# samholt/NeuralLaplaceControl

Hardware: AMD Instinct MI355X
Metric: MPPI planning steps/sec (16384 samples, H=40) (higher is better)
Workload: dtype f64

## Files before the change

neurallaplacecontrol_amd/csrc/abi_ctx.hip:

```cpp
#include "nlc_host.h"

using namespace nlc;
using namespace nlc::host;

namespace nlc {
namespace host {

thread_local std::string g_create_error;

bool gru_use_coop(const nlc_ctx* c, int64_t n_windows) {
  if (c->opt.gru_coop >= 0) return c->opt.gru_coop != 0;
  if (c->g == 128) return true;
  return n_windows <= (c->g == 32 ? 8192 : 50000);
}

void prof_flush(nlc_ctx* c) {
  for (auto& p : c->prof) {
    for (auto& ev : p.pending) {
      hipEventSynchronize(ev.second);
      float ms = 0.f;
      hipEventElapsedTime(&ms, ev.first, ev.second);
      p.total_ms += ms;
      c->event_pool.push_back(ev.first);
      c->event_pool.push_back(ev.second);
// ... 157 lines not shown
    if (value < 0 || value > 3) return fail(c, NLC_ERR_BAD_ARG, "fused_inline must be 0, 1 (= 3), or the bit mask 1 weights | 2 sampling");
    c->opt.fused_inline = (int)value == 1 ? 3 : (int)value;
  } else if (n == "fused_spin_limit") {
    if (value < 1 || value > 4.0e9) return fail(c, NLC_ERR_BAD_ARG, "fused_spin_limit must be in 1 .. 4e9");
    c->opt.fused_spin_limit = (int64_t)value;
  } else if (n == "linear_fused") {
    c->opt.linear_fused = value != 0.0;
  } else if (n == "test_lin_coeff_scale") {
    c->opt.test_lin_coeff_scale = value;
    c->has_mppi = false;
  } else if (n == "fused_keep_sync") {
    c->opt.fused_keep_sync = value != 0.0;
  } else if (n == "fused_test_drop_tile") {
    if (value < -1) return fail(c, NLC_ERR_BAD_ARG, "fused_test_drop_tile must be >= -1");
    c->opt.fused_test_drop_tile = (int)value;
  } else if (n == "fused_roll_cap") {
    if (value < 0) return fail(c, NLC_ERR_BAD_ARG, "fused_roll_cap must be >= 0 (0 = auto)");
    c->opt.fused.roll_cap = (int)value;
  } else if (n == "fused_chain_first_tiles") {
    if (value < -1 || value > 64) return fail(c, NLC_ERR_BAD_ARG, "fused_chain_first_tiles must be in -1..64 (-1 = auto)");
    c->opt.fused.chain_first_tiles = (int)value;
  } else if (n == "fused_partner_tiles") {
    if (value < -2 || value > 64) return fail(c, NLC_ERR_BAD_ARG, "fused_partner_tiles must be in -2..64 (-2 = auto, -1 = never)");
    c->opt.fused.partner_tiles = (int)value;
  } else if (n == "repfunc_split") {
    if (value != 0 && value != 1) return fail(c, NLC_ERR_BAD_ARG, "repfunc_split must be 0 or 1");
    c->opt.repfunc_split = (int)value;
  } else if (n == "gru_coop") {
    if (value != 0 && value != 1 && value != -1) return fail(c, NLC_ERR_BAD_ARG, "gru_coop must be -1 (auto), 0 or 1");
    c->opt.gru_coop = (int)value;
  } else if (n == "gru_prefix") {
    if (value != 0 && value != 1 && value != -1) return fail(c, NLC_ERR_BAD_ARG, "gru_prefix must be -1 (auto), 0 or 1");
    c->opt.gru_prefix = (int)value;
  } else if (n == "gru_gemm") {
    if (value != 0 && value != 1) return fail(c, NLC_ERR_BAD_ARG, "gru_gemm must be 0 (FP64 MFMA) or 1 (int8-sliced)");
    c->opt.gru_gemm = (int)value;
    if (c->has_model) c->gru.use_i8 = (c->gru.i8_stream != nullptr && value == 1) ? 1 : 0;
  } else if (n == "dbg_gap_us") {
    if (value < 0 || value > 1.0e5) return fail(c, NLC_ERR_BAD_ARG, "dbg_gap_us must be in 0 .. 1e5");
    c->opt.dbg_gap_us = value;
  } else if (n == "dbg_l2_mb") {
    if (value < 0 || value > 4096) return fail(c, NLC_ERR_BAD_ARG, "dbg_l2_mb must be in 0 .. 4096");
    c->opt.dbg_l2_mb = value;
  } else if (n == "fused_max_samples") {
    if (value < 0) return fail(c, NLC_ERR_BAD_ARG, "fused_max_samples must be >= 0");
    c->opt.fused_max_samples = (int64_t)value;
  } else {
    return fail(c, NLC_ERR_BAD_ARG, "unknown option: " + n);
  }
  return NLC_OK;
}

extern "C" int nlc_get_stat(nlc_ctx* c, const char* name, double* out) {
  if (!c) return NLC_ERR_BAD_ARG;
  if (!name || !out) return fail(c, NLC_ERR_BAD_ARG, "NULL stat name / out");
  const std::string n(name);
  if (n == "rollout_body") *out = (double)c->last_body;
  else if (n == "fused_timeouts") *out = (double)c->fused.timeouts;
  else if (n == "fused_fallbacks") *out = (double)c->fused.fallbacks;
  else if (n == "fused_lost") *out = c->fused.lost ? 1.0 : 0.0;
  else if (n == "last_giveup_command") *out = (double)c->fused.last_giveup_command;
  else if (n == "commands") *out = (double)c->commands;
  else if (n == "comm_world") *out = c->comm ? (double)c->comm_world : 0.0;
  else if (n == "comm_rank") *out = c->comm ? (double)c->comm_rank : -1.0;
  else if (n == "fused_blocks_per_cu") *out = (double)c->fused.blocks_per_cu;
  else if (n == "fused_spin_limit") *out = (double)c->opt.fused_spin_limit;
  else if (n == "model_nt3") *out = c->has_model ? (double)c->net.nt3 : 0.0;
  else if (n == "gru_gemm") *out = (c->has_model && c->gru.use_i8) ? 1.0 : 0.0;
  else if (n == "gru_prefix") *out = c->prefix.last_used ? 1.0 : 0.0;
  else if (n.rfind("gru_prefix_windows_l", 0) == 0 && n.size() == 21 && n[20] >= '0' && n[20] <= '4') {
    *out = 0.0;
    if (c->prefix.last_used && c->prefix.lists) {
      unsigned cnt[nlc::prefix::kLists] = {0};
      NLC_HIP(c, hipStreamSynchronize(c->stream));
      NLC_HIP(c, hipMemcpy(cnt, c->prefix.lists, sizeof(cnt), hipMemcpyDeviceToHost));
      *out = (double)cnt[n[20] - '0'];
    }
  } else if (n == "gru_prefix_table_tiles") {
    *out = 0.0;
    if (c->prefix.last_used && c->prefix.lists) {
      unsigned cnt[nlc::prefix::kLists] = {0};
      NLC_HIP(c, hipStreamSynchronize(c->stream));
      NLC_HIP(c, hipMemcpy(cnt, c->prefix.lists, sizeof(cnt), hipMemcpyDeviceToHost));
      for (int l = 1; l < nlc::prefix::n_lists(c->prefix.last_B); ++l) *out += (double)((cnt[l] + 15u) / 16u);
    }
  } else if (n == "latents_offset") *out = (c->has_mppi && c->pd.dynamics == NLC_DYN_NL) ? (double)ws_layout(c).pa : -1.0;
  else if (n == "gru_i8_launches") *out = (double)nlc::gru_i8_launch_count();
  else return fail(c, NLC_ERR_BAD_ARG, "unknown stat: " + n);
  return NLC_OK;
}

extern "C" int nlc_synchronize(nlc_ctx* c) {
  if (!c) return NLC_ERR_BAD_ARG;
  NLC_HIP(c, hipStreamSynchronize(c->stream));
  return NLC_OK;
}

extern "C" int nlc_device_info(nlc_ctx* c, char* name, int name_len, int* cus, int* mhz, double* gib) {
  if (!c) return NLC_ERR_BAD_ARG;
  if (name && name_len > 0) {
    std::snprintf(name, name_len, "%s (%s)", c->prop.name, c->prop.gcnArchName);
  }
  if (cus) *cus = c->prop.multiProcessorCount;
  if (mhz) *mhz = c->prop.clockRate / 1000;
  if (gib) *gib = (double)c->prop.totalGlobalMem / (1024.0 * 1024.0 * 1024.0);
  return NLC_OK;
}

extern "C" int nlc_profile_enable(nlc_ctx* c, int on) {
  if (!c) return NLC_ERR_BAD_ARG;
  if (!on) prof_flush(c);
  c->profiling = on != 0;
  return NLC_OK;
}
extern "C" int nlc_profile_reset(nlc_ctx* c) {
  if (!c) return NLC_ERR_BAD_ARG;
// ... 19 lines not shown
```

neurallaplacecontrol_amd/csrc/abi_planner.hip:

```cpp
#include "nlc_host.h"

using namespace nlc;
using namespace nlc::host;

extern "C" int nlc_mppi_configure(nlc_ctx* c, const nlc_mppi_desc* d) {
  if (!c) return NLC_ERR_BAD_ARG;
  NLC_GUARD_BEGIN
  if (!d) return fail(c, NLC_ERR_BAD_ARG, "NULL desc");
  if (d->K < 1 || d->T < 1 || d->K_global < d->K || d->k_offset < 0 || d->k_offset + d->K > d->K_global)
    return fail(c, NLC_ERR_BAD_SHAPE, "bad K / K_global / k_offset / T");
  if (d->nu < 1 || d->nu > NLC_MAX_NU) return fail(c, NLC_ERR_UNSUPPORTED, "nu must be 1 or 2");
  if (d->d < 1 || (d->d > NLC_MAX_D && d->dynamics != NLC_DYN_EXTERNAL)) return fail(c, NLC_ERR_BAD_SHAPE, "bad nx");
  if (d->B < 1) return fail(c, NLC_ERR_BAD_SHAPE, "action_buffer needs at least one row");
  if (!(d->lambda_ > 0.0) || d->u_scale == 0.0) return fail(c, NLC_ERR_BAD_ARG, "lambda_ must be > 0, u_scale != 0");
  if (d->u_per_command < 1 || d->u_per_command > d->T) return fail(c, NLC_ERR_BAD_ARG, "bad u_per_command");
  if (d->E < 0 || d->E > 65535) return fail(c, NLC_ERR_BAD_ARG, "episodes E must be in [0, 65535]");
  const int E = d->E < 1 ? 1 : d->E;
  if ((double)E * (double)d->K * d->T * d->nu > 2.0e9)
    return fail(c, NLC_ERR_BAD_SHAPE, "E*K*T*nu exceeds the planner's index range");
  const bool env_free = d->cost_external &&
                        (d->dynamics == NLC_DYN_NL || d->dynamics == NLC_DYN_DTRNN || d->dynamics == NLC_DYN_NODE) &&
                        d->env == -1;
  if (!env_free && (d->env < 0 || d->env > NLC_ENV_CARTPOLE_NOTRIG)) return fail(c, NLC_ERR_UNSUPPORTED, "unknown env id");
  static const int env_d[4] = {5, 3, 6, 4}, env_nu[4] = {1, 1, 2, 1};
// ... 162 lines not shown
  wa.nblk = c->nblk;
  return wa;
}

int finish_rollout_costs(nlc_ctx* c, const nlc_mppi_buffers* buf, bool in_body) {
  const nlc_mppi_desc& d = c->pd;
  if (d.cost_external) return NLC_OK;
  if (cost_variant_of(d) && !in_body) {
    if (!buf->states) return fail(c, NLC_ERR_BAD_ARG, "this rollout body evaluates a cost_variant on buf->states");
    VariantCostArgs v{d.K * d.E, d.T, d.nu, d.d, d.env, cost_variant_of(d), d.u_scale, buf->states, buf->perturbed, buf->cost_total};
    ProfScope ps(c, "variant_cost_kernel");
    NLC_HIP(c, launch_variant_cost(v, c->stream));
  }
  return run_weights(c, buf);
}

int run_weights(nlc_ctx* c, const nlc_mppi_buffers* buf) {
  WeightArgs wa = make_weight_args(c, buf);
  if (c->last_body == 3 && buf->workspace && c->pd.dynamics == NLC_DYN_NL)
    wa.gave_up = reinterpret_cast<const unsigned*>((const double*)buf->workspace + ws_layout(c).sync) + kFusedTimeout;
  ProfScope ps(c, "weight_kernels");
  NLC_HIP(c, launch_weights(wa, c->stream));
  return NLC_OK;
}

int launch_shift_perturb(nlc_ctx* c, RolloutCall& call) {
  PerturbArgs& p = call.p;
  p.fused_shift = (int64_t)p.K * p.T > 0;
  if (!p.fused_shift) {
    ProfScope ps(c, "shift_U_kernel");
    NLC_HIP(c, launch_shift_U(p, c->stream));
  }
  ProfScope ps(c, "perturb_kernel");
  NLC_HIP(c, launch_perturb(p, c->stream));
  return NLC_OK;
}

SampleCostArgs sample_cost_args(const nlc_ctx* c, const RolloutCall& call) {
  const nlc_mppi_desc& d = c->pd;
  SampleCostArgs a{};
  a.K = call.KE;
  a.Kep = d.K;
  a.T = d.T;
  a.nu = d.nu;
  a.env = (d.cost_external || cost_variant_of(d)) ? -1 : d.env;
  a.state_per_sample = call.state_per_sample;
  a.state0 = call.state_dev;
  a.perturbed = call.buf->perturbed;
  a.noise = call.buf->noise;
  a.U = c->U[c->ucur];
  for (int i = 0; i < NLC_MAX_NU * NLC_MAX_NU; ++i) a.sigma_inv[i] = d.noise_sigma_inv[i];
  a.lambda_ = d.lambda_;
  a.u_scale = d.u_scale;
  a.noise_abs_cost = d.noise_abs_cost;
  a.states = call.buf->states;
  a.cost_total = call.buf->cost_total;
  return a;
}

PerturbArgs perturb_args(const nlc_ctx* c, const nlc_mppi_buffers* buf, int rng, uint64_t seed, uint64_t counter) {
  const nlc_mppi_desc& d = c->pd;
  PerturbArgs p{};
  p.K = d.K * d.E;
  p.Kep = d.K;
  p.E = d.E;
  p.K_global = d.K_global;
  p.k_offset = d.k_offset;
// ... 390 lines not shown
```

neurallaplacecontrol_amd/csrc/abi_planner_nl.hip:

```cpp
#include "nlc_host.h"

using namespace nlc;
using namespace nlc::host;

namespace {

__global__ void dbg_spin_kernel(unsigned long long ticks_100mhz) {
  const unsigned long long t0 = __builtin_amdgcn_s_memrealtime();
  while (__builtin_amdgcn_s_memrealtime() - t0 < ticks_100mhz) __builtin_amdgcn_s_sleep(8);
}
__global__ void dbg_touch_kernel(const double* __restrict__ p, size_t n, double* __restrict__ sink) {
  double acc = 0.0;
  for (size_t i = (size_t)blockIdx.x * blockDim.x + threadIdx.x; i < n; i += (size_t)gridDim.x * blockDim.x) acc += p[i];
  if (acc == 12345.678) *sink = acc;
}
int dbg_between(nlc_ctx* c) {
  if (c->opt.dbg_gap_us > 0.0) hipLaunchKernelGGL(dbg_spin_kernel, dim3(1), dim3(64), 0, c->stream, (unsigned long long)(c->opt.dbg_gap_us * 100.0));
  if (c->opt.dbg_l2_mb > 0.0) {
    const size_t bytes = (size_t)(c->opt.dbg_l2_mb * 1048576.0);
    const size_t n = bytes / 8 + 1;
    if (c->dbg_scratch_n < n) {
      if (int rc = hold_doubles(c, c->dbg_scratch, n, nullptr, &c->dbg_scratch_n)) return rc;
      NLC_HIP(c, hipMemsetAsync(c->dbg_scratch, 0, n * sizeof(double), c->stream));
    }
// ... 296 lines not shown
  fc.n_enc = s.n_enc;
  fc.roll_cap = s.roll_cap;
  fc.adaptive_q8 = s.adaptive_q8;
  fc.pool_wgs = s.pool_wgs;
  fc.chain_first_tiles = s.chain_first_tiles;
  fc.partner_tiles = s.partner_tiles;
  fc.spin_limit = (unsigned)c->opt.fused_spin_limit;
  fc.test_drop_tile = c->opt.fused_test_drop_tile;
  fc.inline_weights = (c->opt.fused_inline & 1) && d.E == 1 && !d.cost_external;
  fc.inline_perturb = (c->opt.fused_inline & 2) && d.E == 1 && inline_inputs && rng == 1 && d.B <= kFusedMaxInlineB;
  unsigned* sync_words = reinterpret_cast<unsigned*>(ws + w.sync);
  const size_t n_sync = fused_sync_words(d.T, KE);
  if (fc.inline_perturb) {
    if (c->fused.sync_clean_ws != buf->workspace) NLC_HIP(c, hipMemsetAsync(sync_words, 0, n_sync * sizeof(unsigned), c->stream));
  } else {
    p.zero_words = sync_words;
    p.n_zero_words = (int64_t)n_sync;
    if (int rc = launch_shift_perturb(c, call)) return rc;
  }
  c->fused.sync_clean_ws = nullptr;
  c->fused.sync_dirty = true;
  c->fused.last.fused = true;
  c->last_body = 3;
  f.p = p;
  if (fc.inline_weights) f.w = make_weight_args(c, buf);
  {
    ProfScope ps(c, "nl_plan_fused_kernel");
    NLC_HIP(c, launch_nl_plan_fused(f, c->g, s.grid, s.built, c->stream));
  }
  *weights_done = fc.inline_weights != 0;
  return NLC_OK;
}

int gru_prefix_begin(nlc_ctx* c, RolloutCall& call, const GruArgs& g, int64_t N, int chunks, bool* use, GruPrefixArgs* px) {
  *use = false;
  if (c->opt.gru_prefix == 0) return NLC_OK;
  GruPrefixState& ps = c->prefix;
  const char* why = ps.why_not;
  if (!why && ps.last_B != g.B) why = "gru_prefix: the table was built for another action-buffer length";
  if (!why && chunks != 1) why = "gru_prefix: not with the encoder in horizon chunks (horizon_chunks)";
  if (!why && gru_use_coop(c, N)) why = "gru_prefix: this launch takes the cooperative encoder (gru_coop)";
  if (!why && g.use_i8) why = "gru_prefix: the FP64 encoder only (gru_gemm is 1)";
  if (!why) why = prefix::out_of_scope(g.nact, g.nin, 1, g.B, N, true);
  if (why) return c->opt.gru_prefix == 1 ? fail(c, NLC_ERR_UNSUPPORTED, why) : NLC_OK;
  const int64_t stride = (N + 63) / 64 * 64;
  const size_t need = 64 + (size_t)prefix::kLists * (size_t)stride / 2;
  if (need > ps.lists_n) {
    NLC_HIP(c, hipStreamSynchronize(c->stream));
    if (int rc = hold_doubles(c, ps.lists, need, nullptr, &ps.lists_n)) return rc;
  }
  double* base = c->arena.base + ps.arena_off;
  px->table = base;
  px->out_tab = base + (size_t)prefix::kEntries * 2 * c->g;
  px->products = base + gru_prefix_products_off(c->g);
  px->counts = reinterpret_cast<unsigned*>(ps.lists);
  px->lists = reinterpret_cast<unsigned*>(ps.lists + 64);
  px->list_stride = stride;
  px->img_max = ps.img_max;
  px->img_min = ps.img_min;
  call.p.zero_words = px->counts;
  call.p.n_zero_words = 16;
  *use = true;
  return NLC_OK;
}

int rollout_nl_two_launch(nlc_ctx* c, RolloutCall& call, GruArgs& g, RolloutArgs& r, int variant) {
  const nlc_mppi_desc& d = c->pd;
  const int64_t KE = call.KE;
  bool use_prefix = false;
  GruPrefixArgs px{};
  {
    const int chunks = plan::horizon_chunks((variant != 2 && KE > 8192 && d.E == 1) ? c->opt.horizon_chunks : 1, d.T).C;
    if (int rc = gru_prefix_begin(c, call, g, KE * d.T, chunks, &use_prefix, &px)) return rc;
  }
  if (int rc2 = nlc::host::launch_shift_perturb(c, call)) return rc2;
  const plan::Chunks ck = plan::horizon_chunks((variant != 2 && KE > 8192 && d.E == 1) ? c->opt.horizon_chunks : 1, d.T);
  const int C = ck.C, Tc = ck.Tc;
  if (C == 1) {
    g.t0 = 0;
    g.Tc = d.T;
    g.N = KE * d.T;
    if (use_prefix) {
      {
        ProfScope ps(c, "gru_prefix_index_kernel");
        NLC_HIP(c, launch_gru_prefix_index(g, px, c->stream));
      }
      ProfScope ps(c, "gru_encode_kernel");
      NLC_HIP(c, launch_gru_encode_prefix(g, px, c->g, c->stream));
      c->prefix.last_used = true;
    } else {
      ProfScope ps(c, "gru_encode_kernel");
      NLC_HIP(c, launch_gru_encode(g, c->g, c->stream, gru_use_coop(c, g.N)));
    }
    if (c->opt.dbg_gap_us > 0.0 || c->opt.dbg_l2_mb > 0.0)
      if (int rc3 = dbg_between(c)) return rc3;
    r.t_begin = 0;
    r.t_end = d.T;
    ProfScope ps(c, "nl_rollout_kernel");
    NLC_HIP(c, launch_nl_rollout(r, c->stream, variant));
  } else {
    if (int rc = gru_encode_chunks(c, g, KE, C, Tc, false, 0u)) return rc;
    for (int ch = 0; ch < C; ++ch) {
      r.t_begin = ch * Tc;
      r.t_end = (r.t_begin + Tc <= d.T) ? r.t_begin + Tc : d.T;
      if (r.t_begin >= r.t_end) break;
      NLC_HIP(c, hipStreamWaitEvent(c->stream, c->side.ev_gru[ch], 0));
      ProfScope ps(c, "nl_rollout_kernel");
      NLC_HIP(c, launch_nl_rollout(r, c->stream, 1));
    }
  }
  return NLC_OK;
}

}

int nlc::host::gru_prefix_configure(nlc_ctx* c) {
  const nlc_mppi_desc& d = c->pd;
  GruPrefixState& ps = c->prefix;
  ps.last_B = d.B;
  ps.last_used = false;
  const double img[2] = {prefix::bound_image(d.u_max[0], d.u_scale), prefix::bound_image(d.u_min[0], d.u_scale)};
  bool finite = true;
// ... 109 lines not shown
```

neurallaplacecontrol_amd/csrc/kernels_gru.hip:

```cpp
#include "nlc_device.h"
#include "nlc_gru_prefix.h"
#include "nlc_gru_tile.h"
#include "nlc_kernels.h"

namespace nlc {

template <int G>
__global__ __launch_bounds__(256, G <= 64 ? 2 : 1) void gru_encode_kernel(const GruArgs a) {
  constexpr int KS = G / 4;
  const int lane = threadIdx.x & 63, wave = threadIdx.x >> 6;
  const int q = lane >> 4, c = lane & 15;
  const int64_t w = ((int64_t)blockIdx.x * 4 + wave) * 16 + c;
  const bool valid = w < a.N;
  const int64_t wc = valid ? w : a.N - 1;
  int64_t kk = 0;
  int tt = 0;
  if (a.mode == 1) {
    kk = wc / a.Tc;
    tt = a.t0 + (int)(wc - kk * a.Tc);
  }
  __shared__ double Hs[4][2][KS * 64];
  const double o = gru_encode_tile<G>(a, lane, wc, kk, tt, Hs[wave][0], Hs[wave][1]);
  if (valid && q < 2) {
    const int64_t wo = (a.mode == 1) ? kk * a.T + tt : w;
// ... 105 lines not shown
  __syncthreads();
  if (threadIdx.x <= prefix::kMaxLen) {
    const unsigned n = cnt[threadIdx.x];
    base[threadIdx.x] = n ? atomicAdd(px.counts + threadIdx.x, n) : 0u;
    cnt[threadIdx.x] = 0u;
  }
  __syncthreads();
#pragma unroll
  for (int it = 0; it < kIndexPerThread; ++it) {
    const int64_t w = w0 + it * 256;
    const int len = (int)(cls[it] & 7u);
    for (int l = 0; l < nl; ++l) {
      const unsigned long long m = __ballot(len == l);
      if (m == 0ull) continue;
      const int leader = __ffsll((long long)m) - 1;
      unsigned b = 0u;
      if (lane == leader) b = atomicAdd(&cnt[l], (unsigned)__popcll(m));
      b = (unsigned)__shfl((int)b, leader);
      if (len == l) {
        const unsigned pos = base[l] + b + (unsigned)__popcll(m & ((1ull << lane) - 1ull));
        if ((int64_t)pos < px.list_stride) px.lists[(int64_t)l * px.list_stride + pos] = (unsigned)w | ((cls[it] >> 3) << prefix::kPatternShift);
      }
    }
  }
}

template <int G>
__global__ __launch_bounds__(256, G <= 64 ? 2 : 1) void gru_encode_prefix_kernel(const GruArgs a, const GruPrefixArgs px) {
  constexpr int KS = G / 4;
  const int lane = threadIdx.x & 63;
  const int wave = __builtin_amdgcn_readfirstlane(threadIdx.x >> 6);
  const int q = lane >> 4, c = lane & 15;
  const int nl = prefix::n_lists(a.B);
  int64_t tile = (int64_t)blockIdx.x * 4 + wave;
  int len = 0;
  unsigned n = 0u;
  for (; len < nl; ++len) {
    n = px.counts[len];
    if ((int64_t)n > px.list_stride) n = (unsigned)px.list_stride;
    const int64_t nt = ((int64_t)n + 15) / 16;
    if (tile < nt) break;
    tile -= nt;
  }
  if (len == nl) return;
  const int64_t idx = tile * 16 + c;
  const bool valid = idx < (int64_t)n;
  const unsigned e = px.lists[(int64_t)len * px.list_stride + (valid ? idx : (int64_t)n - 1)];
  int64_t w = (int64_t)(e & ((1u << prefix::kPatternShift) - 1u));
  if (w >= a.N) w = a.N - 1;
  const int64_t kk = w / a.Tc;
  const int tt = a.t0 + (int)(w - kk * a.Tc);
  __shared__ double Hs[4][2][KS * 64];
  double* prod = nullptr;
  if (len > 0) {
    const int pattern = (int)(e >> prefix::kPatternShift) & ((1 << len) - 1);
    const int entry = prefix::entry_index(len, pattern);
    const double* ent = px.table + (size_t)entry * 2 * G;
    prod = px.products + prefix::products_entry_offset(entry, G);
#pragma unroll
    for (int ks = 0; ks < KS; ++ks) {
      Hs[wave][0][ks * 64 + lane] = ent[4 * ks + q];
      Hs[wave][1][ks * 64 + lane] = ent[G + 4 * ks + q];
    }
  }
  const double o = gru_encode_tile<G, kTileFromTable>(a, lane, w, kk, tt, Hs[wave][0], Hs[wave][1], len, -1, prod);
  if (valid && q < 2) a.out[(kk * a.T + tt) * 2 + q] = o;
// ... 121 lines not shown
```

neurallaplacecontrol_amd/csrc/kernels_mppi.hip:

```cpp
#include "nlc_device.h"
#include "nlc_env_dev.h"
#include "nlc_envcost.h"
#include "nlc_kernels.h"
#include "nlc_mppi_dev.h"

namespace nlc {

__global__ void shift_U_kernel(const PerturbArgs a) {
  const int n = a.T * a.nu;
  const double* Uo = a.U_old + (int64_t)blockIdx.x * n;
  double* Un = a.U_new + (int64_t)blockIdx.x * n;
  for (int i = threadIdx.x; i < n; i += blockDim.x) {
    const int t = i / a.nu, j = i - t * a.nu;
    Un[i] = (t + 1 < a.T) ? Uo[i + a.nu] : a.u_init[j];
  }
  if (blockIdx.x == 0) {
    for (int i = threadIdx.x; i < a.n_state_in; i += blockDim.x) a.state_dst[i] = a.state_in[i];
    for (int i = threadIdx.x; i < a.n_abuf_in; i += blockDim.x) a.abuf_dst[i] = a.abuf_in[i];
  }
}
hipError_t launch_shift_U(const PerturbArgs& a, hipStream_t s) {
  hipLaunchKernelGGL(shift_U_kernel, dim3((unsigned)a.E), dim3(128), 0, s, a);
  return hipGetLastError();
}

__global__ __launch_bounds__(256) void perturb_kernel(const PerturbArgs a) {
  const int64_t total = a.K * a.T;
  for (int64_t i = (int64_t)blockIdx.x * blockDim.x + threadIdx.x; i < a.n_zero_words; i += (int64_t)gridDim.x * blockDim.x)
    a.zero_words[i] = 0u;
  if (a.fused_shift && blockIdx.x == 0) {
    for (int i = threadIdx.x; i < a.n_state_in; i += blockDim.x) a.state_dst[i] = a.state_in[i];
    for (int i = threadIdx.x; i < a.n_abuf_in; i += blockDim.x) a.abuf_dst[i] = a.abuf_in[i];
  }
  for (int64_t idx = (int64_t)blockIdx.x * blockDim.x + threadIdx.x; idx < total;
       idx += (int64_t)gridDim.x * blockDim.x) {
    const int64_t k = idx / a.T;
    const int t = (int)(idx - k * a.T);
    const int64_t e = k / a.Kep;
    const int64_t ke = a.k_offset + (k - e * a.Kep);
    const int64_t kg = e * a.K_global + ke;
    double eps[NLC_MAX_NU];
    if (a.rng) {
      mppi_draw(kg, t, a.seed, a.counter, a.nu, a.mu, a.chol, eps);
    } else {
      for (int i = 0; i < a.nu; ++i) eps[i] = a.noise[idx * a.nu + i];
    }
    const bool null_action = a.sample_null_action && (ke == a.K_global - 1);
    for (int i = 0; i < a.nu; ++i) {
      double U;
      if (a.fused_shift) {
        U = (t + 1 < a.T) ? a.U_old[(e * a.T + t + 1) * a.nu + i] : a.u_init[i];
        if (k == e * a.Kep) a.U_new[(e * a.T + t) * a.nu + i] = U;
      } else {
        U = a.U_new[(e * a.T + t) * a.nu + i];
      }
      const double V = mppi_bound(U, eps[i], null_action, a.u_scale, a.has_bounds, a.u_min[i], a.u_max[i]);
      a.perturbed[idx * a.nu + i] = V;
      a.noise[idx * a.nu + i] = V - U;
      if (a.actions != nullptr) a.actions[idx * a.nu + i] = (a.u_scale * V) / a.u_scale;
    }
  }
}
hipError_t launch_perturb(const PerturbArgs& a, hipStream_t s) {
  const int64_t total = a.K * a.T;
  if (total <= 0) return hipSuccess;
  const int64_t want = (total + 255) / 256;
  const unsigned grid = (unsigned)(want < 4096 ? want : 4096);
  hipLaunchKernelGGL(perturb_kernel, dim3(grid), dim3(256), 0, s, a);
  return hipGetLastError();
}

__global__ __launch_bounds__(256) void weight_tile_kernel(const WeightArgs a) {
  const int lane = threadIdx.x & 63;
  const int64_t b = (int64_t)blockIdx.x * 4 + (threadIdx.x >> 6);
  if (b >= a.nblk) return;
  const int64_t e = blockIdx.y;
  const int64_t ks = b * kWeightTile + (lane & 15);
  const bool valid = ks < a.Kep;
  const double cost = valid ? a.cost[e * a.Kep + ks] : 0.0;
  weight_tile<MemPlain>(a, e, b, lane, cost, valid);
}
__global__ __launch_bounds__(256) void weight_rank_kernel(const WeightArgs a) {
  __shared__ double lds[kWeightRankLds];
  weight_rank<MemPlain>(a, (int64_t)blockIdx.y, lds);
  if (a.gave_up != nullptr && threadIdx.x == 0 && __hip_atomic_load(a.gave_up, __ATOMIC_RELAXED, __HIP_MEMORY_SCOPE_AGENT) != 0u)
    a.partials[(int64_t)blockIdx.y * (2 + a.T * a.nu) + 1] = kPartialInvalidEta;
}
__global__ __launch_bounds__(256) void weight_chunk_kernel(const WeightArgs a) {
  __shared__ double lds[kWeightRankLds];
  const int64_t e = blockIdx.y;
  const int j = blockIdx.x, lane = threadIdx.x & 63, TN = a.T * a.nu;
  const double beta = weight_beta<MemPlain>(a, e, lds);
  for (int i0 = 0; i0 < 1 + TN; i0 += 64) {
    const double c = weight_chunk<MemPlain>(a, e, j, i0, beta, lds);
    if (threadIdx.x < 64 && i0 + lane < 1 + TN) a.chunk_part[(e * gridDim.x + j) * (2 + TN) + 1 + i0 + lane] = c;
  }
  if (threadIdx.x == 0) a.chunk_part[(e * gridDim.x + j) * (2 + TN)] = beta;
}
__global__ __launch_bounds__(128) void weight_final_kernel(const WeightArgs a, int nch) {
#pragma clang fp contract(off)
  const int64_t e = blockIdx.y;
// ... 321 lines not shown
```

neurallaplacecontrol_amd/csrc/nlc_gru_prefix.h:

```cpp
#pragma once
#include <cstdint>

#if defined(__HIPCC__)
#define NLC_PREFIX_HD __host__ __device__
#else
#define NLC_PREFIX_HD
#endif

namespace nlc {
namespace prefix {

constexpr int kMaxLen = 4;
constexpr int kEntries = (2 << kMaxLen) - 1;
constexpr int kLists = kMaxLen + 1;
constexpr int kMaxB = 32;
constexpr int kPatternShift = 27;
constexpr int64_t kMaxWindows = (int64_t)1 << kPatternShift;

NLC_PREFIX_HD inline uint64_t bits_of(double x) {
  uint64_t u;
  __builtin_memcpy(&u, &x, sizeof(u));
  return u;
}
NLC_PREFIX_HD inline double bound_image(double bound, double u_scale) { return bound / u_scale; }
NLC_PREFIX_HD inline int cap(int B) { return B < kMaxLen ? B : kMaxLen; }
NLC_PREFIX_HD inline int n_lists(int B) { return B < kLists ? B : kLists; }
NLC_PREFIX_HD inline int entry_index(int len, int pattern) { return (1 << len) - 1 + pattern; }

struct Class {
  int len, pattern;
};
NLC_PREFIX_HD inline Class classify(const double* row, int t, int B, uint64_t img_max, uint64_t img_min) {
  Class c{0, 0};
  const int L = cap(B);
  for (int s = 0; s < L; ++s) {
    const int i = t + B - 1 - s;
    if (i < B - 1) break;
    const uint64_t v = bits_of(row[i - (B - 1)]);
    if (v == img_max) {
    } else if (v == img_min) {
      c.pattern |= 1 << s;
    } else {
      break;
    }
    c.len = s + 1;
  }
  return c;
}

NLC_PREFIX_HD inline bool starts_tile(int len, int B) { return len >= 1 && len < n_lists(B); }
NLC_PREFIX_HD inline int build_steps(int B) { return B <= kMaxLen ? B : kMaxLen + 1; }
NLC_PREFIX_HD inline int64_t products_doubles(int g) { return (int64_t)(kEntries - 1) * 6 * g; }
NLC_PREFIX_HD inline int64_t products_entry_offset(int entry, int g) { return (int64_t)(entry - 1) * 6 * g; }
NLC_PREFIX_HD inline int products_index(int layer, int j, int set, int q, int r, int g) {
  return (((layer * (g / 16) + j) * 3 + set) * 4 + q) * 4 + r;
}

NLC_PREFIX_HD inline int64_t worst_case_tiles(int64_t N, int B) { return N / 16 + n_lists(B); }

inline const char* out_of_scope(int nu, int nin, int has_bounds, int B, int64_t N, bool images_finite) {
  if (nu != 1 || nin != 1) return "gru_prefix: one action dimension and no time channel only (nu == nin == 1)";
  if (!has_bounds) return "gru_prefix: the planner has no action bounds";
  if (B > kMaxB) return "gru_prefix: action buffers of up to 32 rows only";
  if (N > kMaxWindows) return "gru_prefix: at most 2^27 windows per launch";
  if (!images_finite) return "gru_prefix: a bound's normalised image is not finite";
  return nullptr;
}

}
}
```

neurallaplacecontrol_amd/csrc/nlc_host.h:

```cpp
#pragma once
#include <dlfcn.h>
#include <hip/hip_runtime.h>

#include <time.h>

#include <cmath>
#include <cstdio>
#include <cstdlib>
#include <cstring>
#include <stdexcept>
#include <string>
#include <vector>

#include "nlc_gru_prefix.h"
#include "nlc_kernels.h"
#include "nlc_pack.h"
#include "nlc_plan.h"

namespace nlc {
int nl_pick_nt3(int need);

namespace host {

struct ProfEntry {
  std::string name;
  double total_ms = 0.0;
  int64_t launches = 0;
  std::vector<std::pair<hipEvent_t, hipEvent_t>> pending;
};

struct DeviceArena {
  double* base = nullptr;
  size_t n = 0;
  std::vector<double> host;
  size_t push(const std::vector<double>& v) {
    const size_t off = (host.size() + 63) / 64 * 64;
    host.resize(off);
    host.insert(host.end(), v.begin(), v.end());
    return off;
  }
};


struct PlannerOptions {
  int rollout_variant = 0;
  int repfunc_split = 1;
  int gru_coop = -1;
  int gru_prefix = -1;
  int gru_gemm = 0;
  int horizon_chunks = 1;
  int dehoog_gru_chunks = 0;
  int dehoog_gru_lds_pad = 49152;
  int dehoog_chain = -1;
  int dehoog_chain_phases = 3;
  int dehoog_streams = 0;
  int linear_fused = 1;
  int host_spin = 1;
  double host_spin_margin_us = 150.0;
  nlc::plan::FusedKnobs fused;
  int64_t fused_max_samples = 4096;
  int fused_inline = 3;
  int64_t fused_spin_limit = 1 << 18;
  int fused_keep_sync = 0;
  int fused_test_drop_tile = -1;
  double test_lin_coeff_scale = 1.0;
  double dbg_gap_us = 0.0;
  double dbg_l2_mb = 0.0;
};

struct FusedState {
  int blocks_per_cu = -1;
  int blocks_per_cu3 = -1;
  int occ_h = 0;
  bool lost = false;
  int64_t fallbacks = 0;
  int64_t timeouts = 0;
  int64_t last_giveup_command = -1;
  const void* sync_clean_ws = nullptr;
  bool sync_dirty = false;
  struct LastCommand {
// ... 7 lines not shown
    sync_clean_ws = nullptr;
    sync_dirty = false;
    last.valid = false;
  }
  void rearm() { lost = false; }
};

struct DehoogCalib {
  int n = 0, choice = -1, pending = -1, pending_round = 0;
  double t0 = 0.0;
  float ms[3][2] = {{1e30f, 1e30f}, {1e30f, 1e30f}, {1e30f, 1e30f}};
  hipEvent_t ev[2] = {nullptr, nullptr};
  void reset() {
    n = 0;
    choice = pending = -1;
    for (auto& v : ms) v[0] = v[1] = 1e30f;
  }
  void destroy() {
    for (hipEvent_t& e : ev) {
      if (e) hipEventDestroy(e);
      e = nullptr;
    }
  }
};

struct GruPrefixState {
  size_t arena_off = 0;
  const char* why_not = "gru_prefix: planner not configured";
  unsigned long long img_max = 0, img_min = 0;
  double* lists = nullptr;
  size_t lists_n = 0;
  bool last_used = false;
  int last_B = 0;
};

struct HostWait {
  unsigned long long seq = 0;
  double hist_us[8] = {0};
  int hist_n = 0, hist_at = 0;
  double nap_margin_us = 0.0;
  void reset() {
    hist_n = hist_at = 0;
    nap_margin_us = 0.0;
  }
};

struct SideStreams {
  hipStream_t gru_stream = nullptr;
  std::vector<hipEvent_t> ev_gru;
  std::vector<hipStream_t> aux_streams;
  hipEvent_t ev_fork = nullptr;
  std::vector<hipEvent_t> ev_join;
  hipEvent_t stage_ev = nullptr;
  void destroy() {
    if (stage_ev) hipEventDestroy(stage_ev);
    if (ev_fork) hipEventDestroy(ev_fork);
    for (hipEvent_t e : ev_join) hipEventDestroy(e);
    for (hipStream_t s : aux_streams) hipStreamDestroy(s);
    for (hipEvent_t e : ev_gru) hipEventDestroy(e);
    if (gru_stream) hipStreamDestroy(gru_stream);
    *this = SideStreams{};
  }
};

}
}
// ... 203 lines not shown
  const char* (*GetErrorString)(int) = nullptr;
  std::string why;
  bool ok = false;
};
Rccl* rccl();
constexpr int kNcclFloat64 = 8;

bool linear_on_rollout_kernels(const nlc_ctx* c);
struct WsLayout {
  size_t tile_part, chunk_part, pa, state0, abuf, xcarry, ccarry, fre, fim, dx, tconst, rq, sync, total;
};
WsLayout ws_layout(const nlc_ctx* c);
inline unsigned* pin_giveup_word(nlc_ctx* c) { return reinterpret_cast<unsigned*>(c->pinned + c->pin.giveup); }
inline unsigned long long* pin_seq_word(nlc_ctx* c) { return reinterpret_cast<unsigned long long*>(c->pinned + c->pin.seq); }
inline unsigned* pin_merge_status_word(nlc_ctx* c) { return reinterpret_cast<unsigned*>(c->pinned + c->pin.merge_status); }
WeightArgs make_weight_args(nlc_ctx* c, const nlc_mppi_buffers* buf);
int run_weights(nlc_ctx* c, const nlc_mppi_buffers* buf);
inline int cost_variant_of(const nlc_mppi_desc& d) {
  if (d.cost_external || !(d.cost_variant & (NLC_COST_STATE_CONSTRAINT | NLC_COST_CHANGE_GOAL))) return 0;
  return d.cost_variant;
}
template <class A>
void cost_in_body(A& a, const nlc_mppi_desc& d) {
  if (cost_variant_of(d)) {
    a.env = d.env;
    a.cost_variant = cost_variant_of(d);
  }
}
int finish_rollout_costs(nlc_ctx* c, const nlc_mppi_buffers* buf, bool in_body = false);

struct RolloutCall {
  const nlc_mppi_buffers* buf;
  PerturbArgs p;
  WsLayout w;
  double* ws;
  double* state_dev;
  double* abuf_dev;
  int64_t KE;
  int state_per_sample, rng;
  bool inline_inputs;
  bool replay;
};
int launch_shift_perturb(nlc_ctx* c, RolloutCall& call);
SampleCostArgs sample_cost_args(const nlc_ctx* c, const RolloutCall& call);
int rollout_nl(nlc_ctx* c, RolloutCall& call);
int gru_prefix_configure(nlc_ctx* c);
inline size_t gru_prefix_products_off(int g) { return (size_t)nlc::prefix::kEntries * 2 * g + 64 + (size_t)16 * nlc::prefix::kMaxB; }
inline size_t gru_prefix_arena_doubles(int g) {
  return gru_prefix_products_off(g) + (size_t)nlc::prefix::products_doubles(g);
}

}
}
```

neurallaplacecontrol_amd/csrc/nlc_kernels.h:

```cpp
#pragma once
#include <hip/hip_runtime.h>
#include <stdint.h>

#include <climits>
#include <type_traits>

#include "../../include/nlc.h"
#include "nlc_ilt_tile.h"

namespace nlc {

struct IltArgs {
  const double* theta;
  const double* phi;
  const double* t;
  double* x;
  int64_t N;
  int d, S;
  double alpha, log_tol, scale;
  const double* fre;
  const double* fim;
  double t_div;
  int t_stride;
  int rpp, iters;
// ... 75 lines not shown
  const double* perturbed;
  const double* abuf;
  double u_scale;
  int mode, T;
  int t0, Tc;
  int64_t Kep;
  int64_t N;
  int B, nin;
  int nact;
  double mean[NLC_MAX_NIN], std[NLC_MAX_NIN];
  const double* Wih0p;
  const double* Whh0p;
  const double* Wih1p;
  const double* Whh1p;
  const double* Wop;
  const double* bhn0;
  const double* brz1;
  const double* bin1;
  const double* bhn1;
  double bo[2];
  double* out;
  int use_i8;
  const signed char* i8_stream;
};
hipError_t launch_gru_encode(const GruArgs& a, int g, hipStream_t s, bool coop = false, unsigned lds_pad_bytes = 0);
hipError_t launch_gru_encode_i8(const GruArgs& a, hipStream_t s);
unsigned long long gru_i8_launch_count();
struct GruPrefixArgs {
  double* table;
  double* out_tab;
  double* products;
  unsigned* lists;
  unsigned* counts;
  int64_t list_stride;
  unsigned long long img_max, img_min;
};
hipError_t launch_gru_prefix_table(const GruArgs& a, const GruPrefixArgs& px, int g, hipStream_t s);
hipError_t launch_gru_prefix_index(const GruArgs& a, const GruPrefixArgs& px, hipStream_t s);
hipError_t launch_gru_encode_prefix(const GruArgs& a, const GruPrefixArgs& px, int g, hipStream_t s);

struct SampleCostArgs {
  int64_t K;
  int64_t Kep;
  int T;
  int nu;
  int env;
  int state_per_sample;
  const double* state0;
  const double* perturbed;
  const double* noise;
  const double* U;
  double sigma_inv[NLC_MAX_NU * NLC_MAX_NU];
  double lambda_;
  double u_scale;
  int noise_abs_cost;
  double* states;
  double* cost_total;
  SampleCostArgs part(int64_t o, int64_t n, int d) const {
    SampleCostArgs v = *this;
    v.K = n;
    if (n < K) v.Kep = n;
    v.state0 = state0 + (state_per_sample ? o * d : 0);
    v.perturbed = perturbed + o * T * nu;
    v.noise = noise + o * T * nu;
    v.states = states ? states + o * T * d : nullptr;
    v.cost_total = cost_total + o;
// ... 237 lines not shown
  uint64_t seed;
  double* s0;
  double* a0;
  double* sn;
  double* ts;
};
hipError_t launch_synth(const SynthArgs& a, hipStream_t s);

constexpr int kMaxInlineAbuf = 32;
struct PerturbArgs {
  int64_t K, Kep, K_global, k_offset;
  int T, nu, E;
  const double* U_old;
  double* U_new;
  double* noise;
  double* perturbed;
  double* actions;
  double u_scale;
  int has_bounds, sample_null_action, rng;
  double u_min[NLC_MAX_NU], u_max[NLC_MAX_NU], u_init[NLC_MAX_NU], mu[NLC_MAX_NU];
  double chol[NLC_MAX_NU * NLC_MAX_NU];
  uint64_t seed, counter;
  int n_state_in, n_abuf_in;
  double* state_dst;
  double* abuf_dst;
  double state_in[NLC_MAX_D];
  double abuf_in[kMaxInlineAbuf];
  unsigned* zero_words;
  int64_t n_zero_words;
  int fused_shift;
};
hipError_t launch_shift_U(const PerturbArgs& a, hipStream_t s);
hipError_t launch_perturb(const PerturbArgs& a, hipStream_t s);

struct WeightArgs {
  int64_t Kep;
  int T, nu, E;
  double lambda_;
  const double* cost;
  const double* noise;
  double* tile_part;
  double* chunk_part;
  double* partials;
  int nblk;
  const unsigned* gave_up;
};
constexpr double kPartialInvalidEta = -1.0;
constexpr int kWeightTile = 16;
inline int weight_tiles(int64_t Kep) { return (int)((Kep + kWeightTile - 1) / kWeightTile); }
hipError_t launch_weights(const WeightArgs& a, hipStream_t s);

struct MergeArgs {
  int64_t Kep;
  int T, nu, G, rank, u_per_command, E;
  double lambda_, u_scale;
  const double* gathered;
  double* U;
  double* cost_nz;
  double* omega;
  double* action;
  double* action_pinned;
  double* beta_eta;
  const double* cost;
  unsigned* zero_words;
  int64_t n_zero_words;
  unsigned long long* seq_pinned;
// ... 107 lines not shown
```

Before: 271.7.

## Fuse GRU prefix indexing into perturb kernel with double-buffered counters

Adds a perturb_classify kernel that draws the perturbed actions, computes each element's clip class in shared memory, and builds the GRU prefix window lists in the same pass. This removes the separate gru_prefix_index launch and its re-read of the perturbed buffer. The list counters are double-buffered so the encode kernel clears the next row's counts, which avoids a memset or zeroing step on most calls. The cost is a 1024-thread block with a serial backward scan and extra atomics. The fused path only applies when rng=1, nu=1 and T fits in a block.

```diff
diff --git a/neurallaplacecontrol_amd/csrc/abi_ctx.hip b/neurallaplacecontrol_amd/csrc/abi_ctx.hip
--- a/neurallaplacecontrol_amd/csrc/abi_ctx.hip
+++ b/neurallaplacecontrol_amd/csrc/abi_ctx.hip
@@ -213,6 +213,9 @@
   } else if (n == "gru_prefix") {
     if (value != 0 && value != 1 && value != -1) return fail(c, NLC_ERR_BAD_ARG, "gru_prefix must be -1 (auto), 0 or 1");
     c->opt.gru_prefix = (int)value;
+  } else if (n == "gru_prefix_fused_index") {
+    if (value != 0 && value != 1) return fail(c, NLC_ERR_BAD_ARG, "gru_prefix_fused_index must be 0 or 1");
+    c->opt.gru_prefix_fused_index = (int)value;
   } else if (n == "gru_gemm") {
     if (value != 0 && value != 1) return fail(c, NLC_ERR_BAD_ARG, "gru_gemm must be 0 (FP64 MFMA) or 1 (int8-sliced)");
     c->opt.gru_gemm = (int)value;
@@ -249,12 +252,13 @@
   else if (n == "model_nt3") *out = c->has_model ? (double)c->net.nt3 : 0.0;
   else if (n == "gru_gemm") *out = (c->has_model && c->gru.use_i8) ? 1.0 : 0.0;
   else if (n == "gru_prefix") *out = c->prefix.last_used ? 1.0 : 0.0;
+  else if (n == "gru_prefix_fused_index") *out = (double)c->prefix.fused_index;
   else if (n.rfind("gru_prefix_windows_l", 0) == 0 && n.size() == 21 && n[20] >= '0' && n[20] <= '4') {
     *out = 0.0;
     if (c->prefix.last_used && c->prefix.lists) {
       unsigned cnt[nlc::prefix::kLists] = {0};
       NLC_HIP(c, hipStreamSynchronize(c->stream));
-      NLC_HIP(c, hipMemcpy(cnt, c->prefix.lists, sizeof(cnt), hipMemcpyDeviceToHost));
+      NLC_HIP(c, hipMemcpy(cnt, reinterpret_cast<const unsigned*>(c->prefix.lists) + 32 * c->prefix.last_row, sizeof(cnt), hipMemcpyDeviceToHost));
       *out = (double)cnt[n[20] - '0'];
     }
   } else if (n == "gru_prefix_table_tiles") {
@@ -262,7 +266,7 @@
     if (c->prefix.last_used && c->prefix.lists) {
       unsigned cnt[nlc::prefix::kLists] = {0};
       NLC_HIP(c, hipStreamSynchronize(c->stream));
-      NLC_HIP(c, hipMemcpy(cnt, c->prefix.lists, sizeof(cnt), hipMemcpyDeviceToHost));
+      NLC_HIP(c, hipMemcpy(cnt, reinterpret_cast<const unsigned*>(c->prefix.lists) + 32 * c->prefix.last_row, sizeof(cnt), hipMemcpyDeviceToHost));
       for (int l = 1; l < nlc::prefix::n_lists(c->prefix.last_B); ++l) *out += (double)((cnt[l] + 15u) / 16u);
     }
   } else if (n == "latents_offset") *out = (c->has_mppi && c->pd.dynamics == NLC_DYN_NL) ? (double)ws_layout(c).pa : -1.0;
diff --git a/neurallaplacecontrol_amd/csrc/abi_planner.hip b/neurallaplacecontrol_amd/csrc/abi_planner.hip
--- a/neurallaplacecontrol_amd/csrc/abi_planner.hip
+++ b/neurallaplacecontrol_amd/csrc/abi_planner.hip
@@ -218,7 +218,10 @@
     NLC_HIP(c, launch_shift_U(p, c->stream));
   }
   ProfScope ps(c, "perturb_kernel");
-  NLC_HIP(c, launch_perturb(p, c->stream));
+  if (call.ix.lists != nullptr)
+    NLC_HIP(c, launch_perturb_classify(p, call.ix, c->stream));
+  else
+    NLC_HIP(c, launch_perturb(p, c->stream));
   return NLC_OK;
 }
 
diff --git a/neurallaplacecontrol_amd/csrc/abi_planner_nl.hip b/neurallaplacecontrol_amd/csrc/abi_planner_nl.hip
--- a/neurallaplacecontrol_amd/csrc/abi_planner_nl.hip
+++ b/neurallaplacecontrol_amd/csrc/abi_planner_nl.hip
@@ -352,8 +352,10 @@
   return NLC_OK;
 }
 
-int gru_prefix_begin(nlc_ctx* c, RolloutCall& call, const GruArgs& g, int64_t N, int chunks, bool* use, GruPrefixArgs* px) {
+int gru_prefix_begin(nlc_ctx* c, RolloutCall& call, const GruArgs& g, int64_t N, int chunks, bool* use, GruPrefixArgs* px,
+                     bool* fused_index) {
   *use = false;
+  *fused_index = false;
   if (c->opt.gru_prefix == 0) return NLC_OK;
   GruPrefixState& ps = c->prefix;
   const char* why = ps.why_not;
@@ -368,18 +370,41 @@
   if (need > ps.lists_n) {
     NLC_HIP(c, hipStreamSynchronize(c->stream));
     if (int rc = hold_doubles(c, ps.lists, need, nullptr, &ps.lists_n)) return rc;
+    ps.clean_row = -1;
   }
   double* base = c->arena.base + ps.arena_off;
   px->table = base;
   px->out_tab = base + (size_t)prefix::kEntries * 2 * c->g;
   px->products = base + gru_prefix_products_off(c->g);
-  px->counts = reinterpret_cast<unsigned*>(ps.lists);
+  const int row = ps.row;
+  ps.row ^= 1;
+  ps.last_row = row;
+  px->counts = reinterpret_cast<unsigned*>(ps.lists) + 32 * row;
+  px->counts_next = reinterpret_cast<unsigned*>(ps.lists) + 32 * (row ^ 1);
   px->lists = reinterpret_cast<unsigned*>(ps.lists + 64);
   px->list_stride = stride;
   px->img_max = ps.img_max;
   px->img_min = ps.img_min;
-  call.p.zero_words = px->counts;
-  call.p.n_zero_words = 16;
+  const PerturbArgs& p = call.p;
+  const int rows = (p.rng == 1 && p.nu == 1 && p.K > 0 && p.T > 0 && p.K * p.T == N) ? classify_rows(p.T) : 0;
+  if (c->opt.gru_prefix_fused_index != 0 && rows >= 1) {
+    if (ps.clean_row != row) NLC_HIP(c, hipMemsetAsync(px->counts, 0, 8 * sizeof(unsigned), c->stream));
+    ps.clean_row = -1;
+    PerturbIndexArgs& ix = call.ix;
+    ix.lists = px->lists;
+    ix.counts = px->counts;
+    ix.list_stride = stride;
+    ix.out_tab = px->out_tab;
+    ix.out = g.out;
+    ix.img_max = ps.img_max;
+    ix.img_min = ps.img_min;
+    ix.B = g.B;
+    ix.rows = rows;
+    *fused_index = true;
+  } else {
+    call.p.zero_words = px->counts;
+    call.p.n_zero_words = 16;
+  }
   *use = true;
   return NLC_OK;
 }
@@ -387,11 +412,11 @@
 int rollout_nl_two_launch(nlc_ctx* c, RolloutCall& call, GruArgs& g, RolloutArgs& r, int variant) {
   const nlc_mppi_desc& d = c->pd;
   const int64_t KE = call.KE;
-  bool use_prefix = false;
+  bool use_prefix = false, fused_index = false;
   GruPrefixArgs px{};
   {
     const int chunks = plan::horizon_chunks((variant != 2 && KE > 8192 && d.E == 1) ? c->opt.horizon_chunks : 1, d.T).C;
-    if (int rc = gru_prefix_begin(c, call, g, KE * d.T, chunks, &use_prefix, &px)) return rc;
+    if (int rc = gru_prefix_begin(c, call, g, KE * d.T, chunks, &use_prefix, &px, &fused_index)) return rc;
   }
   if (int rc2 = nlc::host::launch_shift_perturb(c, call)) return rc2;
   const plan::Chunks ck = plan::horizon_chunks((variant != 2 && KE > 8192 && d.E == 1) ? c->opt.horizon_chunks : 1, d.T);
@@ -401,13 +426,16 @@
     g.Tc = d.T;
     g.N = KE * d.T;
     if (use_prefix) {
-      {
+      if (fused_index) {
+        c->prefix.fused_index += 1;
+      } else {
         ProfScope ps(c, "gru_prefix_index_kernel");
         NLC_HIP(c, launch_gru_prefix_index(g, px, c->stream));
       }
       ProfScope ps(c, "gru_encode_kernel");
       NLC_HIP(c, launch_gru_encode_prefix(g, px, c->g, c->stream));
       c->prefix.last_used = true;
+      c->prefix.clean_row = c->prefix.last_row ^ 1;
     } else {
       ProfScope ps(c, "gru_encode_kernel");
       NLC_HIP(c, launch_gru_encode(g, c->g, c->stream, gru_use_coop(c, g.N)));
diff --git a/neurallaplacecontrol_amd/csrc/kernels_gru.hip b/neurallaplacecontrol_amd/csrc/kernels_gru.hip
--- a/neurallaplacecontrol_amd/csrc/kernels_gru.hip
+++ b/neurallaplacecontrol_amd/csrc/kernels_gru.hip
@@ -161,6 +161,7 @@
   const int wave = __builtin_amdgcn_readfirstlane(threadIdx.x >> 6);
   const int q = lane >> 4, c = lane & 15;
   const int nl = prefix::n_lists(a.B);
+  if (blockIdx.x == 0 && threadIdx.x < 8) px.counts_next[threadIdx.x] = 0u;
   int64_t tile = (int64_t)blockIdx.x * 4 + wave;
   int len = 0;
   unsigned n = 0u;
diff --git a/neurallaplacecontrol_amd/csrc/kernels_mppi.hip b/neurallaplacecontrol_amd/csrc/kernels_mppi.hip
--- a/neurallaplacecontrol_amd/csrc/kernels_mppi.hip
+++ b/neurallaplacecontrol_amd/csrc/kernels_mppi.hip
@@ -1,6 +1,7 @@
 #include "nlc_device.h"
 #include "nlc_env_dev.h"
 #include "nlc_envcost.h"
+#include "nlc_gru_prefix.h"
 #include "nlc_kernels.h"
 #include "nlc_mppi_dev.h"
 
@@ -24,41 +25,47 @@
   return hipGetLastError();
 }
 
+__device__ __forceinline__ double perturb_element(const PerturbArgs& a, int64_t idx, int64_t k, int t) {
+  const int64_t e = k / a.Kep;
+  const int64_t ke = a.k_offset + (k - e * a.Kep);
+  const int64_t kg = e * a.K_global + ke;
+  double eps[NLC_MAX_NU];
+  if (a.rng) {
+    mppi_draw(kg, t, a.seed, a.counter, a.nu, a.mu, a.chol, eps);
+  } else {
+    for (int i = 0; i < a.nu; ++i) eps[i] = a.noise[idx * a.nu + i];
+  }
+  const bool null_action = a.sample_null_action && (ke == a.K_global - 1);
+  double V0 = 0.0;
+  for (int i = 0; i < a.nu; ++i) {
+    double U;
+    if (a.fused_shift) {
+      U = (t + 1 < a.T) ? a.U_old[(e * a.T + t + 1) * a.nu + i] : a.u_init[i];
+      if (k == e * a.Kep) a.U_new[(e * a.T + t) * a.nu + i] = U;
+    } else {
+      U = a.U_new[(e * a.T + t) * a.nu + i];
+    }
+    const double V = mppi_bound(U, eps[i], null_action, a.u_scale, a.has_bounds, a.u_min[i], a.u_max[i]);
+    a.perturbed[idx * a.nu + i] = V;
+    a.noise[idx * a.nu + i] = V - U;
+    if (a.actions != nullptr) a.actions[idx * a.nu + i] = (a.u_scale * V) / a.u_scale;
+    if (i == 0) V0 = V;
+  }
+  return V0;
+}
+__device__ __forceinline__ void perturb_stage_inputs(const PerturbArgs& a) {
+  for (int i = threadIdx.x; i < a.n_state_in; i += blockDim.x) a.state_dst[i] = a.state_in[i];
+  for (int i = threadIdx.x; i < a.n_abuf_in; i += blockDim.x) a.abuf_dst[i] = a.abuf_in[i];
+}
 __global__ __launch_bounds__(256) void perturb_kernel(const PerturbArgs a) {
   const int64_t total = a.K * a.T;
   for (int64_t i = (int64_t)blockIdx.x * blockDim.x + threadIdx.x; i < a.n_zero_words; i += (int64_t)gridDim.x * blockDim.x)
     a.zero_words[i] = 0u;
-  if (a.fused_shift && blockIdx.x == 0) {
-    for (int i = threadIdx.x; i < a.n_state_in; i += blockDim.x) a.state_dst[i] = a.state_in[i];
-    for (int i = threadIdx.x; i < a.n_abuf_in; i += blockDim.x) a.abuf_dst[i] = a.abuf_in[i];
-  }
+  if (a.fused_shift && blockIdx.x == 0) perturb_stage_inputs(a);
   for (int64_t idx = (int64_t)blockIdx.x * blockDim.x + threadIdx.x; idx < total;
        idx += (int64_t)gridDim.x * blockDim.x) {
     const int64_t k = idx / a.T;
-    const int t = (int)(idx - k * a.T);
-    const int64_t e = k / a.Kep;
-    const int64_t ke = a.k_offset + (k - e * a.Kep);
-    const int64_t kg = e * a.K_global + ke;
-    double eps[NLC_MAX_NU];
-    if (a.rng) {
-      mppi_draw(kg, t, a.seed, a.counter, a.nu, a.mu, a.chol, eps);
-    } else {
-      for (int i = 0; i < a.nu; ++i) eps[i] = a.noise[idx * a.nu + i];
-    }
-    const bool null_action = a.sample_null_action && (ke == a.K_global - 1);
-    for (int i = 0; i < a.nu; ++i) {
-      double U;
-      if (a.fused_shift) {
-        U = (t + 1 < a.T) ? a.U_old[(e * a.T + t + 1) * a.nu + i] : a.u_init[i];
-        if (k == e * a.Kep) a.U_new[(e * a.T + t) * a.nu + i] = U;
-      } else {
-        U = a.U_new[(e * a.T + t) * a.nu + i];
-      }
-      const double V = mppi_bound(U, eps[i], null_action, a.u_scale, a.has_bounds, a.u_min[i], a.u_max[i]);
-      a.perturbed[idx * a.nu + i] = V;
-      a.noise[idx * a.nu + i] = V - U;
-      if (a.actions != nullptr) a.actions[idx * a.nu + i] = (a.u_scale * V) / a.u_scale;
-    }
+    perturb_element(a, idx, k, (int)(idx - k * a.T));
   }
 }
 hipError_t launch_perturb(const PerturbArgs& a, hipStream_t s) {
@@ -67,6 +74,86 @@
   const int64_t want = (total + 255) / 256;
   const unsigned grid = (unsigned)(want < 4096 ? want : 4096);
   hipLaunchKernelGGL(perturb_kernel, dim3(grid), dim3(256), 0, s, a);
+  return hipGetLastError();
+}
+
+__global__ __launch_bounds__(kClassifyThreads) void perturb_classify_kernel(const PerturbArgs a, const PerturbIndexArgs ix) {
+  __shared__ unsigned char cls_s[kClassifyGroups][kClassifyThreads];
+  __shared__ unsigned cnt[8], base[8];
+  const int tid = threadIdx.x, lane = tid & 63;
+  const int nl = prefix::n_lists(ix.B);
+  if (tid < 8) cnt[tid] = 0u;
+  if (blockIdx.x == 0) perturb_stage_inputs(a);
+  const int row = tid / a.T, t = tid - row * a.T;
+  const int64_t k0 = (int64_t)blockIdx.x * kClassifyGroups * ix.rows + row;
+#pragma unroll
+  for (int it = 0; it < kClassifyGroups; ++it) {
+    const int64_t k = k0 + (int64_t)it * ix.rows;
+    int cls = prefix::kNotClipped;
+    if (row < ix.rows && k < a.K) cls = prefix::clip_class(perturb_element(a, k * a.T + t, k, t), ix.img_max, ix.img_min);
+    cls_s[it][tid] = (unsigned char)cls;
+  }
+  __syncthreads();
+  unsigned code[kClassifyGroups];
+#pragma unroll
+  for (int it = 0; it < kClassifyGroups; ++it) {
+    const int64_t k = k0 + (int64_t)it * ix.rows;
+    int len = 7, pattern = 0;
+    if (row < ix.rows && k < a.K) {
+      const prefix::Class c = prefix::classify_classes(cls_s[it] + tid, t, ix.B);
+      len = c.len;
+      pattern = c.pattern;
+      if (len == ix.B) {
+        const double* o = ix.out_tab + prefix::entry_index(len, pattern) * 2;
+        ix.out[(k * a.T + t) * 2 + 0] = o[0];
+        ix.out[(k * a.T + t) * 2 + 1] = o[1];
+      }
+    }
+    code[it] = (unsigned)len | ((unsigned)pattern << 3);
+    for (int l = 0; l <= prefix::kMaxLen; ++l) {
+      const unsigned long long m = __ballot(len == l);
+      if (m != 0ull && lane == __ffsll((long long)m) - 1) atomicAdd(&cnt[l], (unsigned)__popcll(m));
+    }
+  }
+  __syncthreads();
+  if (tid < 2) {
+    const unsigned long long n = (unsigned long long)cnt[2 * tid] | ((unsigned long long)cnt[2 * tid + 1] << 32);
+    const unsigned long long b = n ? atomicAdd(reinterpret_cast<unsigned long long*>(ix.counts) + tid, n) : 0ull;
+    base[2 * tid] = (unsigned)b;
+    base[2 * tid + 1] = (unsigned)(b >> 32);
+    cnt[2 * tid] = 0u;
+    cnt[2 * tid + 1] = 0u;
+  } else if (tid == 2) {
+    const unsigned n = cnt[4];
+    base[4] = n ? atomicAdd(ix.counts + 4, n) : 0u;
+    cnt[4] = 0u;
+  }
+  __syncthreads();
+#pragma unroll
+  for (int it = 0; it < kClassifyGroups; ++it) {
+    const int64_t idx = (k0 + (int64_t)it * ix.rows) * a.T + t;
+    const int len = (int)(code[it] & 7u);
+    for (int l = 0; l < nl; ++l) {
+      const unsigned long long m = __ballot(len == l);
+      if (m == 0ull) continue;
+      const int leader = __ffsll((long long)m) - 1;
+      unsigned b = 0u;
+      if (lane == leader) b = atomicAdd(&cnt[l], (unsigned)__popcll(m));
+      b = (unsigned)__shfl((int)b, leader);
+      if (len == l) {
+        const unsigned pos = base[l] + b + (unsigned)__popcll(m & ((1ull << lane) - 1ull));
+        if ((int64_t)pos < ix.list_stride) ix.lists[(int64_t)l * ix.list_stride + pos] = (unsigned)idx | ((code[it] >> 3) << prefix::kPatternShift);
+      }
+    }
+  }
+}
+int classify_rows(int T) { return T > 0 ? kClassifyThreads / T : 0; }
+hipError_t launch_perturb_classify(const PerturbArgs& a, const PerturbIndexArgs& ix, hipStream_t s) {
+  if (a.K <= 0 || a.T <= 0) return hipSuccess;
+  if (ix.lists == nullptr || ix.rows < 1 || (int64_t)ix.rows * a.T > kClassifyThreads || a.nu != 1 || !a.rng || !a.fused_shift)
+    return hipErrorInvalidValue;
+  const int64_t per = (int64_t)ix.rows * kClassifyGroups;
+  hipLaunchKernelGGL(perturb_classify_kernel, dim3((unsigned)((a.K + per - 1) / per)), dim3(kClassifyThreads), 0, s, a, ix);
   return hipGetLastError();
 }
 
diff --git a/neurallaplacecontrol_amd/csrc/nlc_gru_prefix.h b/neurallaplacecontrol_amd/csrc/nlc_gru_prefix.h
--- a/neurallaplacecontrol_amd/csrc/nlc_gru_prefix.h
+++ b/neurallaplacecontrol_amd/csrc/nlc_gru_prefix.h
@@ -30,19 +30,31 @@
 struct Class {
   int len, pattern;
 };
+enum { kNotClipped = 0, kClippedMax = 1, kClippedMin = 2 };
+NLC_PREFIX_HD inline int clip_class(double stored, uint64_t img_max, uint64_t img_min) {
+  const uint64_t v = bits_of(stored);
+  return v == img_max ? kClippedMax : (v == img_min ? kClippedMin : kNotClipped);
+}
+NLC_PREFIX_HD inline Class classify_classes(const unsigned char* newest, int t, int B) {
+  Class c{0, 0};
+  const int L = cap(B);
+  for (int s = 0; s < L && s <= t; ++s) {
+    const int cls = newest[-s];
+    if (cls == kNotClipped) break;
+    if (cls == kClippedMin) c.pattern |= 1 << s;
+    c.len = s + 1;
+  }
+  return c;
+}
 NLC_PREFIX_HD inline Class classify(const double* row, int t, int B, uint64_t img_max, uint64_t img_min) {
   Class c{0, 0};
   const int L = cap(B);
   for (int s = 0; s < L; ++s) {
     const int i = t + B - 1 - s;
     if (i < B - 1) break;
-    const uint64_t v = bits_of(row[i - (B - 1)]);
-    if (v == img_max) {
-    } else if (v == img_min) {
-      c.pattern |= 1 << s;
-    } else {
-      break;
-    }
+    const int cls = clip_class(row[i - (B - 1)], img_max, img_min);
+    if (cls == kNotClipped) break;
+    if (cls == kClippedMin) c.pattern |= 1 << s;
     c.len = s + 1;
   }
   return c;
diff --git a/neurallaplacecontrol_amd/csrc/nlc_host.h b/neurallaplacecontrol_amd/csrc/nlc_host.h
--- a/neurallaplacecontrol_amd/csrc/nlc_host.h
+++ b/neurallaplacecontrol_amd/csrc/nlc_host.h
@@ -46,6 +46,7 @@
   int rollout_variant = 0;
   int repfunc_split = 1;
   int gru_coop = -1;
+  int gru_prefix_fused_index = 1;
   int gru_prefix = -1;
   int gru_gemm = 0;
   int horizon_chunks = 1;
@@ -119,6 +120,10 @@
   size_t lists_n = 0;
   bool last_used = false;
   int last_B = 0;
+  int row = 0;
+  int last_row = 0;
+  int clean_row = -1;
+  unsigned long long fused_index = 0;
 };
 
 struct HostWait {
@@ -388,6 +393,7 @@
 struct RolloutCall {
   const nlc_mppi_buffers* buf;
   PerturbArgs p;
+  PerturbIndexArgs ix;
   WsLayout w;
   double* ws;
   double* state_dev;
diff --git a/neurallaplacecontrol_amd/csrc/nlc_kernels.h b/neurallaplacecontrol_amd/csrc/nlc_kernels.h
--- a/neurallaplacecontrol_amd/csrc/nlc_kernels.h
+++ b/neurallaplacecontrol_amd/csrc/nlc_kernels.h
@@ -131,6 +131,7 @@
   double* products;
   unsigned* lists;
   unsigned* counts;
+  unsigned* counts_next;
   int64_t list_stride;
   unsigned long long img_max, img_min;
 };
@@ -434,6 +435,20 @@
 };
 hipError_t launch_shift_U(const PerturbArgs& a, hipStream_t s);
 hipError_t launch_perturb(const PerturbArgs& a, hipStream_t s);
+constexpr int kClassifyThreads = 1024;
+constexpr int kClassifyGroups = 4;
+struct PerturbIndexArgs {
+  unsigned* lists;
+  unsigned* counts;
+  int64_t list_stride;
+  const double* out_tab;
+  double* out;
+  unsigned long long img_max, img_min;
+  int B;
+  int rows;
+};
+int classify_rows(int T);
+hipError_t launch_perturb_classify(const PerturbArgs& a, const PerturbIndexArgs& ix, hipStream_t s);
 
 struct WeightArgs {
   int64_t Kep;
```

Result: no change. 272.7 (median of 6 runs) (+0.4%).
